# saguirregaray1/walkai-nos

Measured on AMD Instinct MI355X. Metric: aggregate GPU utilization % + schedulable pods/node, mixed fractional-GPU load, higher is better.
Workload: dtype fp32

## Files before the change

### csrc/attn_wide.hip

```cpp
#include <hip/hip_runtime.h>

#include "pin.h"
#include "x3_common.h"

#include <utility>

namespace {

template <class F, int... Q>
__device__ __forceinline__ void x3w_slots(F& f, std::integer_sequence<int, Q...>) {
  (f(std::integral_constant<int, Q>{}), ...);
}

#ifndef NOS_X3W_FENCE
#define NOS_X3W_FENCE 1
#endif
__device__ __forceinline__ f32x16 x3_step(int k, const bf16x8& a0, const bf16x8& a1, const bf16x8& a2,
                                          const bf16x8& b0, const bf16x8& b1, const bf16x8& b2, const f32x16& d) {
  switch (k) {
    case 0: return __builtin_amdgcn_mfma_f32_32x32x16_bf16(a2, b0, d, 0, 0, 0);
    case 1: return __builtin_amdgcn_mfma_f32_32x32x16_bf16(a1, b1, d, 0, 0, 0);
    case 2: return __builtin_amdgcn_mfma_f32_32x32x16_bf16(a0, b2, d, 0, 0, 0);
    case 3: return __builtin_amdgcn_mfma_f32_32x32x16_bf16(a1, b0, d, 0, 0, 0);
    case 4: return __builtin_amdgcn_mfma_f32_32x32x16_bf16(a0, b1, d, 0, 0, 0);
    default: return __builtin_amdgcn_mfma_f32_32x32x16_bf16(a0, b0, d, 0, 0, 0);
  }
}

template <bool FDIV = false>
__global__ __launch_bounds__(256, 1) void attn_fwd_x3w(const float* __restrict__ qkv, float* __restrict__ out,
                                                       __bf16* __restrict__ outp, float* __restrict__ part_o,
                                                       float* __restrict__ part_ml, int B, int T, int H, int h0,
                                                       int Ht, float scale_log2e, int Pk, int* __restrict__ cnt,
                                                       int q0, int Tq) {
  constexpr int G = 8;
  __shared__ __attribute__((aligned(16))) __bf16 lds_k[2 * 3 * XK_PLANE];
  __shared__ __attribute__((aligned(16))) __bf16 lds_v[2 * 3 * XV_PLANE];
  __shared__ int s_last;
  const int P = Pk & 0x3fffff;
  const PinnedBlock pb = pinned_block(unsigned(Pk >> 22) & 0xffu);
  if (pb.id < 0 || pb.id >= P) return;
  const int w = (Pk >> 30) ? pb.id : xcd_major_n(pb.id, P, pb.nx);
  const int NK = (T + 31) / 32, QT = (Tq + 31) / 32, QG = (QT + G - 1) / G;
  const long long U = (long long)B * H * QG * NK;
  const float rP = FDIV ? 1.f / float(P) : 0.f, rNK = FDIV ? 1.f / float(NK) : 0.f;
  const float rQG = FDIV ? 1.f / float(QG) : 0.f, rH = FDIV ? 1.f / float(H) : 0.f;
  long long u = FDIV ? udiv23(w * U, P, rP) : sk_begin(w, U, P);
  const long long u1 = FDIV ? udiv23((w + 1) * U, P, rP) : sk_begin(w + 1, U, P);
  const int D = Ht * HD, ld = 3 * D;
  const int tid = threadIdx.x, lane = tid & 63;
  const int wv = __builtin_amdgcn_readfirstlane(tid >> 6);
  const int j = lane & 31, hf = lane >> 5;
  const int lrow = tid >> 3, lch = tid & 7;
  const int gi = lane & 15, gg = lane >> 4;
  const int vtr = (4 * hf + (gi >> 2)) * XV_STR + 16 * (gg & 1) + 4 * (gi & 3);
  bool first = true;
  while (u < u1) {
    const long long grp = FDIV ? udiv23(u, NK, rNK) : u / NK;
    const int kb0 = int(u - grp * NK);
    const int kb1 = int(min<long long>(NK, kb0 + (u1 - u)));
    const int nb = kb1 - kb0;
    const long long gq = FDIV ? udiv23(grp, QG, rQG) : grp / QG;
    const int qg = int(grp - gq * QG);
    const long long bq = FDIV ? udiv23(gq, H, rH) : gq / H;
    const int head = h0 + int(gq - bq * H);
    const int b = int(bq);
    const float* basef = qkv + size_t(b) * T * ld;
    const int qtA = qg * G + 2 * wv, qtB = qtA + 1;
    const bool activeA = qtA < QT, activeB = qtB < QT;

    bf16x8 qa[3][4], qb[3][4];
    {
      const float* qpa = basef + size_t(q0 + min(qtA * 32 + j, Tq - 1)) * ld + head * HD + 8 * hf;
      const float* qpb = basef + size_t(q0 + min(qtB * 32 + j, Tq - 1)) * ld + head * HD + 8 * hf;
#pragma unroll
      for (int s = 0; s < 4; ++s) {
        const f32x4 alo = *reinterpret_cast<const f32x4*>(qpa + 16 * s);
        const f32x4 ahi = *reinterpret_cast<const f32x4*>(qpa + 16 * s + 4);
        const f32x4 blo = *reinterpret_cast<const f32x4*>(qpb + 16 * s);
        const f32x4 bhi = *reinterpret_cast<const f32x4*>(qpb + 16 * s + 4);
        split3(f32x8{alo[0], alo[1], alo[2], alo[3], ahi[0], ahi[1], ahi[2], ahi[3]}, qa[0][s], qa[1][s], qa[2][s]);
        split3(f32x8{blo[0], blo[1], blo[2], blo[3], bhi[0], bhi[1], bhi[2], bhi[3]}, qb[0][s], qb[1][s], qb[2][s]);
      }
#pragma unroll
      for (int p = 0; p < 3; ++p)
#pragma unroll
        for (int s = 0; s < 4; ++s) asm volatile("" : "+a"(qa[p][s]), "+a"(qb[p][s]));
    }
    const float* kgf = basef + D + head * HD + 8 * lch;
    const float* vgf = basef + 2 * D + head * HD + 8 * lch;
    f32x4 fk0, fk1, fv0, fv1;
    auto fetch_k = [&](int blk) {
      const size_t r = size_t(min(blk * 32 + lrow, T - 1)) * ld;
      fk0 = *reinterpret_cast<const f32x4*>(kgf + r);
      fk1 = *reinterpret_cast<const f32x4*>(kgf + r + 4);
    };
    auto fetch_v = [&](int blk) {
      const size_t r = size_t(min(blk * 32 + lrow, T - 1)) * ld;
      fv0 = *reinterpret_cast<const f32x4*>(vgf + r);
      fv1 = *reinterpret_cast<const f32x4*>(vgf + r + 4);
    };
    auto stash = [](const f32x4& lo, const f32x4& hi, __bf16* d, int pstride) {
      bf16x8 a0, a1, a2;
      split3(f32x8{lo[0], lo[1], lo[2], lo[3], hi[0], hi[1], hi[2], hi[3]}, a0, a1, a2);
      *reinterpret_cast<bf16x8*>(d) = a0;
      *reinterpret_cast<bf16x8*>(d + pstride) = a1;
      *reinterpret_cast<bf16x8*>(d + 2 * pstride) = a2;
    };
    auto stash_k = [&](int buf) { stash(fk0, fk1, &lds_k[buf * 3 * XK_PLANE + lrow * XK_STR + 8 * lch], XK_PLANE); };
    auto stash_v = [&](int buf) { stash(fv0, fv1, &lds_v[buf * 3 * XV_PLANE + lrow * XV_STR + 8 * lch], XV_PLANE); };
    auto qk_all = [&](f32x16& SA, f32x16& SB, int buf) {
      const __bf16* ks_ = &lds_k[buf * 3 * XK_PLANE + j * XK_STR + 8 * hf];
      SA = f32x16{0};
      SB = f32x16{0};
#pragma unroll
      for (int s = 0; s < 4; ++s) {
        const bf16x8 k0 = *reinterpret_cast<const bf16x8*>(ks_ + 16 * s);
        const bf16x8 k1 = *reinterpret_cast<const bf16x8*>(ks_ + XK_PLANE + 16 * s);
        const bf16x8 k2 = *reinterpret_cast<const bf16x8*>(ks_ + 2 * XK_PLANE + 16 * s);
        SA = mfma_x3(k0, k1, k2, qa[0][s], qa[1][s], qa[2][s], SA);
        SB = mfma_x3(k0, k1, k2, qb[0][s], qb[1][s], qb[2][s], SB);
      }
    };
    auto rowmax = [&](const f32x16& S) {
      float mx = fmaxf(S[0], S[1]);
#pragma unroll
      for (int r = 2; r < 16; ++r) mx = fmaxf(mx, S[r]);
      return half_max(mx);
    };
    __syncthreads();
    fetch_k(kb0);
    fetch_v(kb0);
    stash_k(0);
    stash_v(0);
    fetch_k(kb0 + 1);
    stash_k(1);
    __syncthreads();
    f32x16 oa0 = {0}, oa1 = {0}, ob0 = {0}, ob1 = {0}, sca, scb, sna, snb;
    float ma = -INFINITY, la = 0.f, mb = -INFINITY, lb = 0.f;
    qk_all(sca, scb, 0);
    float mxa = rowmax(sca), mxb = rowmax(scb);
    __syncthreads();
    auto rescale = [&](float mx, float& m, float& l, f32x16& o0, f32x16& o1) {
      if (__builtin_amdgcn_ballot_w64((mx - m) * scale_log2e > 8.f)) {
        const float m_new = fmaxf(m, mx);
        const float alpha = __builtin_amdgcn_exp2f((m - m_new) * scale_log2e);
        l *= alpha;
        o0 *= alpha;
        o1 *= alpha;
        m = m_new;
      }
    };
    auto iter = [&](f32x16& SA, f32x16& SB, f32x16& NA, f32x16& NB, float& mxA, float& mxB, int i) {
      const int blk = kb0 + i;
      if (blk * 32 + 32 > T) {
        asm volatile("; tail block: mask keys >= T" ::: "memory");
#pragma unroll
        for (int r = 0; r < 16; ++r)
          if (blk * 32 + key_of(r, hf) >= T) SA[r] = SB[r] = -INFINITY;
        mxA = rowmax(SA);
        mxB = rowmax(SB);
      }
      rescale(mxA, ma, la, oa0, oa1);
      rescale(mxB, mb, lb, ob0, ob1);
      fetch_k(blk + 2);
      fetch_v(blk + 1);
      const float mcA = ma * scale_log2e, mcB = mb * scale_log2e;
      float psA = 0.f, psB = 0.f;
      const __bf16* ks_ = &lds_k[((i + 1) & 1) * 3 * XK_PLANE + j * XK_STR + 8 * hf];
      const __bf16* vs_ = &lds_v[(i & 1) * 3 * XV_PLANE + vtr];
      bf16x8 kf[2][3], vf[2][2][3];
      uint32_t pw[2][2][3][4];
      float ra[2], rb[2];
      typedef float f32x2v __attribute__((ext_vector_type(2)));
      typedef __bf16 bf16x2v __attribute__((ext_vector_type(2)));
      bf16x2v kh[3][4], vh[3][4];
      f32x2v kr[4], vr[4];
      float mxn = 0.f;
      auto read_k = [&](int s, int slot) {
#pragma unroll
        for (int p = 0; p < 3; ++p) kf[slot][p] = *reinterpret_cast<const bf16x8*>(ks_ + p * XK_PLANE + 16 * s);
      };
      auto read_v = [&](int s2, int dh, int p) {
        const __bf16* a = vs_ + p * XV_PLANE + 16 * s2 * XV_STR + 32 * dh;
        const bf16x4 lo = __builtin_amdgcn_ds_read_tr16_b64_v4bf16((lds_bf16x4*)(a));
        const bf16x4 hi = __builtin_amdgcn_ds_read_tr16_b64_v4bf16((lds_bf16x4*)(a + 8 * XV_STR));
        vf[s2][dh][p] = bf16x8{lo[0], lo[1], lo[2], lo[3], hi[0], hi[1], hi[2], hi[3]};
      };
      auto expo = [&](int t, int r) {
        if (t)
          SB[r] = __builtin_amdgcn_exp2f(fmaf(SB[r], scale_log2e, -mcB));
        else
          SA[r] = __builtin_amdgcn_exp2f(fmaf(SA[r], scale_log2e, -mcA));
      };
      auto addp = [&](int t, int r) {
        if (t)
          psB += SB[r];
        else
          psA += SA[r];
      };
      auto split_a = [&](int t, int s2, int q) {
        const float a = t ? SB[8 * s2 + 2 * q] : SA[8 * s2 + 2 * q];
        const float b = t ? SB[8 * s2 + 2 * q + 1] : SA[8 * s2 + 2 * q + 1];
        const uint32_t ua = __float_as_uint(a), ub = __float_as_uint(b);
        pw[t][s2][0][q] = __builtin_amdgcn_perm(ub, ua, 0x07060302u);
        ra[t] = a - __uint_as_float(ua & 0xffff0000u);
        rb[t] = b - __uint_as_float(ub & 0xffff0000u);
      };
      auto split_b = [&](int t, int s2, int q) {
        const uint32_t ura = __float_as_uint(ra[t]), urb = __float_as_uint(rb[t]);
        pw[t][s2][1][q] = __builtin_amdgcn_perm(urb, ura, 0x07060302u);
        const float sa = ra[t] - __uint_as_float(ura & 0xffff0000u), sb = rb[t] - __uint_as_float(urb & 0xffff0000u);
        pw[t][s2][2][q] = __builtin_amdgcn_perm(__float_as_uint(sb), __float_as_uint(sa), 0x07060302u);
      };
      auto pplane = [&](int t, int s2, int p) {
        return __builtin_bit_cast(bf16x8, (uint4){pw[t][s2][p][0], pw[t][s2][p][1], pw[t][s2][p][2], pw[t][s2][p][3]});
      };
      auto stash_a = [&](bool isv, int q) {
        const f32x4 lo = isv ? fv0 : fk0, hi = isv ? fv1 : fk1;
        const f32x2v x = q < 2 ? f32x2v{lo[2 * q], lo[2 * q + 1]} : f32x2v{hi[2 * q - 4], hi[2 * q - 3]};
        const bf16x2v h0 = __builtin_convertvector(x, bf16x2v);
        const f32x2v r = x - __builtin_convertvector(h0, f32x2v);
        if (isv) vh[0][q] = h0, vr[q] = r;
        else kh[0][q] = h0, kr[q] = r;
      };
      auto stash_b = [&](bool isv, int q) {
        const f32x2v r = isv ? vr[q] : kr[q];
        const bf16x2v h1 = __builtin_convertvector(r, bf16x2v);
        const bf16x2v h2 = __builtin_convertvector(r - __builtin_convertvector(h1, f32x2v), bf16x2v);
        if (isv) vh[1][q] = h1, vh[2][q] = h2;
        else kh[1][q] = h1, kh[2][q] = h2;
      };
      auto stash_w = [&](bool isv) {
        if (isv) {
          __bf16* d = &lds_v[((i + 1) & 1) * 3 * XV_PLANE + lrow * XV_STR + 8 * lch];
#pragma unroll
          for (int p = 0; p < 3; ++p)
            *reinterpret_cast<bf16x8*>(d + p * XV_PLANE) = bf16x8{vh[p][0][0], vh[p][0][1], vh[p][1][0], vh[p][1][1],
                                                                  vh[p][2][0], vh[p][2][1], vh[p][3][0], vh[p][3][1]};
        } else {
          __bf16* d = &lds_k[(i & 1) * 3 * XK_PLANE + lrow * XK_STR + 8 * lch];
#pragma unroll
          for (int p = 0; p < 3; ++p)
            *reinterpret_cast<bf16x8*>(d + p * XK_PLANE) = bf16x8{kh[p][0][0], kh[p][0][1], kh[p][1][0], kh[p][1][1],
                                                                  kh[p][2][0], kh[p][2][1], kh[p][3][0], kh[p][3][1]};
        }
      };
      read_k(0, 0);
      __builtin_amdgcn_sched_barrier(0);
      auto slot = [&](auto qc) {
        constexpr int q = decltype(qc)::value;
        if constexpr (q < 48) {
          constexpr int s = q / 12, t = (q / 6) & 1, k = q % 6;
          const bf16x8* kk = kf[s & 1];
          const bool init = s == 0 && k == 0;
          if (t == 0)
            NA = x3_step(k, kk[0], kk[1], kk[2], qa[0][s], qa[1][s], qa[2][s], init ? f32x16{0} : NA);
          else
            NB = x3_step(k, kk[0], kk[1], kk[2], qb[0][s], qb[1][s], qb[2][s], init ? f32x16{0} : NB);
        } else {
          const int v = q - 48, s2 = v / 24, dh = (v / 12) & 1, t = (v / 6) & 1, k = v % 6;
          const bf16x8* vv = vf[s2][dh];
          const bf16x8 p0 = pplane(t, s2, 0), p1 = pplane(t, s2, 1), p2 = pplane(t, s2, 2);
          if (dh == 0 && t == 0) oa0 = x3_step(k, vv[0], vv[1], vv[2], p0, p1, p2, oa0);
          else if (dh == 0) ob0 = x3_step(k, vv[0], vv[1], vv[2], p0, p1, p2, ob0);
          else if (t == 0) oa1 = x3_step(k, vv[0], vv[1], vv[2], p0, p1, p2, oa1);
          else ob1 = x3_step(k, vv[0], vv[1], vv[2], p0, p1, p2, ob1);
        }
        if constexpr ((q >= 1 && q <= 16) || (q >= 33 && q <= 48)) {
          constexpr int e = q <= 16 ? q - 1 : q - 33;
          addp(e / 8, (q <= 16 ? 0 : 8) + e % 8);
        }
        if (q < 8) expo(0, q);
        else if (q < 16) expo(1, q - 8);
        else if (q < 32) {
          const int t = (q - 16) / 8, pq = ((q - 16) % 8) / 2;
          if (q % 2 == 0) split_a(t, 0, pq); else split_b(t, 0, pq);
        } else if (q < 40) expo(0, q - 32 + 8);
        else if (q < 48) expo(1, q - 40 + 8);
        else if (q < 64) {
          const int t = (q - 48) / 8, pq = ((q - 48) % 8) / 2;
          if (q % 2 == 0) split_a(t, 1, pq); else split_b(t, 1, pq);
        } else if (q == 64) la += half_sum(psA);
        else if (q == 65) lb += half_sum(psB);
        else if (q >= 66 && q < 70) {
          const int c = q - 66;
          float m4 = fmaxf(NA[4 * c], NA[4 * c + 1]);
          m4 = fmaxf(m4, NA[4 * c + 2]);
          m4 = fmaxf(m4, NA[4 * c + 3]);
          mxn = c ? fmaxf(mxn, m4) : m4;
        } else if (q == 70) mxA = half_max(mxn);
        else if (q >= 72 && q < 76) {
          const int c = q - 72;
          float m4 = fmaxf(NB[4 * c], NB[4 * c + 1]);
          m4 = fmaxf(m4, NB[4 * c + 2]);
          m4 = fmaxf(m4, NB[4 * c + 3]);
          mxn = c ? fmaxf(mxn, m4) : m4;
        } else if (q == 76) mxB = half_max(mxn);
        else if (q >= 77 && q < 85) {
          if ((q - 77) % 2 == 0) stash_a(false, (q - 77) / 2); else stash_b(false, (q - 77) / 2);
        } else if (q >= 86 && q < 94) {
          if ((q - 86) % 2 == 0) stash_a(true, (q - 86) / 2); else stash_b(true, (q - 86) / 2);
        }
        if (q == 2 || q == 14 || q == 26) read_k(q / 12 + 1, (q / 12 + 1) & 1);
        if (q >= 29 && q < 41 && (q - 29) % 2 == 0) read_v(0, (q - 29) / 6, (q - 29) / 2 % 3);
        if (q >= 50 && q < 62 && (q - 50) % 2 == 0) read_v(1, (q - 50) / 6, (q - 50) / 2 % 3);
        if (q == 85) stash_w(false);
        if (q == 94) stash_w(true);
        if (NOS_X3W_FENCE) __builtin_amdgcn_sched_barrier(0);
      };
      x3w_slots(slot, std::make_integer_sequence<int, 96>{});
    };
    int i = 0;
    for (; i + 1 < nb; i += 2) {
      iter(sca, scb, sna, snb, mxa, mxb, i);
      __syncthreads();
      iter(sna, snb, sca, scb, mxa, mxb, i + 1);
      __syncthreads();
    }
    if (i < nb) {
      iter(sca, scb, sna, snb, mxa, mxb, i);
      __syncthreads();
    }

    const bool whole = kb0 == 0 && kb1 == NK;
    auto store_tile = [&](int t, const f32x16& o0, const f32x16& o1, float l) {
      const int q = (qg * G + 2 * wv + t) * 32 + j;
      if (q >= Tq) return;
      const float inv = 1.f / l;
      const size_t orow = (size_t(b) * Tq + q) * D + head * HD;
      if (outp) {
        const size_t op = size_t(B) * Tq * D;
#pragma unroll
        for (int r = 0; r < 16; ++r) {
          const int d = key_of(r, hf);
          store_x3(outp, op, orow + d, o0[r] * inv);
          store_x3(outp, op, orow + 32 + d, o1[r] * inv);
        }
      } else {
#pragma unroll
        for (int r = 0; r < 16; ++r) {
          const int d = key_of(r, hf);
          out[orow + d] = o0[r] * inv;
          out[orow + 32 + d] = o1[r] * inv;
        }
      }
    };
    auto finish = [&](bool active, int t, const f32x16& o0, const f32x16& o1, float m, float l) {
      if (!active) return;
      if (whole) {
        store_tile(t, o0, o1, l);
      } else {
        const size_t slot = (size_t(w) * 2 + (first ? 0 : 1)) * G + 2 * wv + t;
        float* po = part_o + slot * (HD * 32);
#pragma unroll
        for (int r = 0; r < 16; ++r) {
          const int d = key_of(r, hf);
          po[d * 32 + j] = o0[r];
          po[(32 + d) * 32 + j] = o1[r];
        }
        if (hf == 0) {
          part_ml[slot * 64 + j] = m * scale_log2e;
          part_ml[slot * 64 + 32 + j] = l;
        }
      }
    };
    finish(activeA, 0, oa0, oa1, ma, la);
    finish(activeB, 1, ob0, ob1, mb, lb);
    if (!whole && cnt) {
      const long long t0 = grp * NK, t1 = t0 + NK;
      const long long wlo = ((t0 + 1) * P + U - 1) / U - 1, whi = (t1 * P + U - 1) / U - 1;
      __threadfence();
      __syncthreads();
      if (tid == 0) {
        int n = 0;
        for (long long x = wlo; x <= whi; ++x) n += (x * U / P != (x + 1) * U / P) ? 1 : 0;
        const int last = atomicAdd(&cnt[grp], 1) == n - 1;
        if (last) atomicExch(&cnt[grp], 0);
        s_last = last;
      }
      __syncthreads();
      if (s_last) {
        __threadfence();
        auto merge = [&](int t) {
          float M = -INFINITY, L = 0.f;
          f32x16 a0 = {0}, a1 = {0};
          for (long long x = wlo; x <= whi; ++x) {
            const long long s0 = x * U / P;
            if (s0 == (x + 1) * U / P) continue;
            const size_t slot = (size_t(x) * 2 + (s0 >= t0 ? 0 : 1)) * G + 2 * wv + t;
            const float mw = part_ml[slot * 64 + j];
            if (mw == -INFINITY) continue;
            const float lw = part_ml[slot * 64 + 32 + j];
            const float* po = part_o + slot * (HD * 32);
            const float Mn = fmaxf(M, mw);
            const float so = __builtin_amdgcn_exp2f(M - Mn), sn = __builtin_amdgcn_exp2f(mw - Mn);
            L = fmaf(lw, sn, L * so);
#pragma unroll
            for (int r = 0; r < 16; ++r) {
              const int d = key_of(r, hf);
              a0[r] = fmaf(po[d * 32 + j], sn, a0[r] * so);
              a1[r] = fmaf(po[(32 + d) * 32 + j], sn, a1[r] * so);
            }
            M = Mn;
          }
          store_tile(t, a0, a1, L);
        };
        if (activeA) merge(0);
        if (activeB) merge(1);
      }
    }
    u += kb1 - kb0;
    first = false;
  }
}

}

int nos_attn_x3w_launch(bool fdiv, dim3 grid, hipStream_t s, const float* qkv, float* out, __bf16* outp,
                        float* part_o, float* part_ml, int B, int T, int H, int h0, int Ht, float scale_log2e,
                        int Pk, int* cnt, int q0, int Tq) {
  if (fdiv)
    hipLaunchKernelGGL(attn_fwd_x3w<true>, grid, dim3(256), 0, s, qkv, out, outp, part_o, part_ml, B, T, H, h0, Ht,
                       scale_log2e, Pk, cnt, q0, Tq);
  else
    hipLaunchKernelGGL(attn_fwd_x3w<false>, grid, dim3(256), 0, s, qkv, out, outp, part_o, part_ml, B, T, H, h0, Ht,
                       scale_log2e, Pk, cnt, q0, Tq);
  return int(hipPeekAtLastError());
}

int nos_attn_x3w_occupancy() {
  int n = 0;
  if (hipOccupancyMaxActiveBlocksPerMultiprocessor(&n, attn_fwd_x3w<true>, 256, 0) != hipSuccess || n <= 0) n = 1;
  return n;
}
```

### csrc/attn_x3.hip

```cpp
#include <hip/hip_runtime.h>

#include "attn_x3.h"
#include "err.h"
#include "pin.h"
#include "x3_common.h"

#include <cmath>
#include <cstdint>
#include <cstdlib>
#include <string>

namespace {


__device__ __forceinline__ void split3_trunc8(const f32x16& acc, int e0, bf16x8& p0, bf16x8& p1, bf16x8& p2) {
  uint32_t w0[4], w1[4], w2[4];
#pragma unroll
  for (int i = 0; i < 4; ++i) {
    const float a = acc[e0 + 2 * i], b = acc[e0 + 2 * i + 1];
    const uint32_t ua = __float_as_uint(a), ub = __float_as_uint(b);
    w0[i] = __builtin_amdgcn_perm(ub, ua, 0x07060302u);
    const float ra = a - __uint_as_float(ua & 0xffff0000u), rb = b - __uint_as_float(ub & 0xffff0000u);
    const uint32_t ura = __float_as_uint(ra), urb = __float_as_uint(rb);
    w1[i] = __builtin_amdgcn_perm(urb, ura, 0x07060302u);
// ... 51 lines not shown
    uint4 pk0, pk1, pk2, pv0, pv1, pv2;
    auto fetch = [&](int blk) {
      const size_t r = size_t(min(blk * 32 + lrow, T - 1)) * ld;
      pk0 = *reinterpret_cast<const uint4*>(kg + r);
      pk1 = *reinterpret_cast<const uint4*>(kg + plane + r);
      pk2 = *reinterpret_cast<const uint4*>(kg + 2 * plane + r);
      pv0 = *reinterpret_cast<const uint4*>(vg + r);
      pv1 = *reinterpret_cast<const uint4*>(vg + plane + r);
      pv2 = *reinterpret_cast<const uint4*>(vg + 2 * plane + r);
    };
    auto stash = [&](int buf) {
      __bf16* kd = &lds_k[buf * 3 * XK_PLANE + lrow * XK_STR + 8 * lch];
      __bf16* vd = &lds_v[buf * 3 * XV_PLANE + lrow * XV_STR + 8 * lch];
      *reinterpret_cast<uint4*>(kd) = pk0;
      *reinterpret_cast<uint4*>(kd + XK_PLANE) = pk1;
      *reinterpret_cast<uint4*>(kd + 2 * XK_PLANE) = pk2;
      *reinterpret_cast<uint4*>(vd) = pv0;
      *reinterpret_cast<uint4*>(vd + XV_PLANE) = pv1;
      *reinterpret_cast<uint4*>(vd + 2 * XV_PLANE) = pv2;
    };
    __syncthreads();
    fetch(kb0);
    stash(0);
    __syncthreads();

    f32x16 o0 = {0}, o1 = {0};
    float m = -INFINITY, l = 0.f;
    for (int blk = kb0; blk < kb1; ++blk) {
      const int buf = (blk - kb0) & 1;
      const bool more = blk + 1 < kb1;
      if (more) fetch(blk + 1);
#define X3_ATTN_BLOCK(MASKED)                                                                        \
  {                                                                                                  \
    const __bf16* ks = &lds_k[buf * 3 * XK_PLANE + j * XK_STR + 8 * hf];                             \
    f32x16 sacc = {0};                                                                               \
    _Pragma("unroll") for (int s = 0; s < 4; ++s) {                                                  \
      const bf16x8 k0 = *reinterpret_cast<const bf16x8*>(ks + 16 * s);                               \
      const bf16x8 k1 = *reinterpret_cast<const bf16x8*>(ks + XK_PLANE + 16 * s);                     \
      const bf16x8 k2 = *reinterpret_cast<const bf16x8*>(ks + 2 * XK_PLANE + 16 * s);                 \
      sacc = mfma_x3(k0, k1, k2, qf[0][s], qf[1][s], qf[2][s], sacc);                                \
    }                                                                                                \
    if (MASKED) {                                                                                    \
      asm volatile("; tail block: mask keys >= T" ::: "memory");           \
      _Pragma("unroll") for (int r = 0; r < 16; ++r) if (blk * 32 + key_of(r, hf) >= T) sacc[r] = -INFINITY; \
    }                                                                                                \
    float mx = fmaxf(sacc[0], sacc[1]);                                                              \
    _Pragma("unroll") for (int r = 2; r < 16; ++r) mx = fmaxf(mx, sacc[r]);                          \
    mx = half_max(mx);                                                          \
    if (__builtin_amdgcn_ballot_w64((mx - m) * scale_log2e > 8.f)) {                                 \
      const float m_new = fmaxf(m, mx);                                                              \
      const float alpha = __builtin_amdgcn_exp2f((m - m_new) * scale_log2e);                         \
      l *= alpha;                                                                                    \
      o0 *= alpha;                                                                                   \
      o1 *= alpha;                                                                                   \
      m = m_new;                                                                                     \
    }                                                                                                \
    const float mc = m * scale_log2e;                                                                \
    float psum = 0.f;                                                                                \
    _Pragma("unroll") for (int r = 0; r < 16; ++r) {                                                 \
      sacc[r] = __builtin_amdgcn_exp2f(fmaf(sacc[r], scale_log2e, -mc));                             \
      psum += sacc[r];                                                                               \
    }                                                                                                \
    psum = half_sum(psum);                                                                \
    l += psum;                                                                                       \
    const __bf16* vs = &lds_v[buf * 3 * XV_PLANE + vtr];                                             \
    _Pragma("unroll") for (int s2 = 0; s2 < 2; ++s2) {                                               \
      bf16x8 p0, p1, p2;                                                                             \
      split3_trunc8(sacc, 8 * s2, p0, p1, p2);                                                       \
      _Pragma("unroll") for (int dh = 0; dh < 2; ++dh) {                                             \
        bf16x8 vf[3];                                                                                \
        _Pragma("unroll") for (int p = 0; p < 3; ++p) {                                              \
          const __bf16* a = vs + p * XV_PLANE + 16 * s2 * XV_STR + 32 * dh;                          \
          const bf16x4 lo = __builtin_amdgcn_ds_read_tr16_b64_v4bf16((lds_bf16x4*)(a));              \
          const bf16x4 hi = __builtin_amdgcn_ds_read_tr16_b64_v4bf16((lds_bf16x4*)(a + 8 * XV_STR)); \
          vf[p] = bf16x8{lo[0], lo[1], lo[2], lo[3], hi[0], hi[1], hi[2], hi[3]};                    \
        }                                                                                            \
        if (dh == 0)                                                                                 \
          o0 = mfma_x3(vf[0], vf[1], vf[2], p0, p1, p2, o0);                                         \
        else                                                                                         \
          o1 = mfma_x3(vf[0], vf[1], vf[2], p0, p1, p2, o1);                                         \
      }                                                                                              \
    }                                                                                                \
  }
      if (active) X3_ATTN_BLOCK(blk * 32 + 32 > T)
#undef X3_ATTN_BLOCK
      if (more) stash(buf ^ 1);
      __syncthreads();
    }

    if (active) {
      if (kb0 == 0 && kb1 == NK) {
        const int q = q0 + j;
        if (q < T) {
          const float inv = 1.f / l;
          const size_t orow = (size_t(b) * T + q) * D + head * HD;
          if (outp) {
            const size_t op = size_t(B) * T * D;
#pragma unroll
            for (int r = 0; r < 16; ++r) {
              const int d = key_of(r, hf);
              store_x3(outp, op, orow + d, o0[r] * inv);
              store_x3(outp, op, orow + 32 + d, o1[r] * inv);
            }
          } else {
#pragma unroll
            for (int r = 0; r < 16; ++r) {
              const int d = key_of(r, hf);
              out[orow + d] = o0[r] * inv;
              out[orow + 32 + d] = o1[r] * inv;
            }
          }
        }
      } else {
        const size_t slot = (size_t(w) * 2 + (first ? 0 : 1)) * 4 + wv;
        float* po = part_o + slot * (HD * 32);
#pragma unroll
        for (int r = 0; r < 16; ++r) {
          const int d = key_of(r, hf);
          po[d * 32 + j] = o0[r];
          po[(32 + d) * 32 + j] = o1[r];
        }
        if (hf == 0) {
          part_ml[slot * 64 + j] = m * scale_log2e;
          part_ml[slot * 64 + 32 + j] = l;
        }
      }
    }
    u += kb1 - kb0;
    first = false;
  }
}

template <int G, bool QW = false, bool F32IN = false, bool PRIO = false, bool FDIV = false>
__global__ __launch_bounds__(64 * G, 8 / G) void attn_fwd_x3p(const __bf16* __restrict__ qkv3, size_t plane,
                                                             float* __restrict__ out, __bf16* __restrict__ outp,
                                                             float* __restrict__ part_o, float* __restrict__ part_ml,
                                                             int B, int T, int H, int h0, int Ht, float scale_log2e,
                                                             int Pk, int qw0, int Tq) {
  static_assert(G == 4 || G == 8, "4 or 8 query tiles per workgroup");
  __shared__ __attribute__((aligned(16))) __bf16 lds_k[2 * 3 * XK_PLANE];
  __shared__ __attribute__((aligned(16))) __bf16 lds_v[2 * 3 * XV_PLANE];
  const int P = Pk & 0x3fffff;
  const PinnedBlock pb = pinned_block(unsigned(Pk >> 22) & 0xffu);
  if (pb.id < 0 || pb.id >= P) return;
  const int w = (Pk >> 30) ? pb.id : xcd_major_n(pb.id, P, pb.nx);
  const int NK = (T + 31) / 32, QT = (Tq + 31) / 32, QG = (QT + G - 1) / G;
  const long long U = (long long)B * H * QG * NK;
  const float rP = FDIV ? 1.f / float(P) : 0.f, rNK = FDIV ? 1.f / float(NK) : 0.f;
  const float rQG = FDIV ? 1.f / float(QG) : 0.f, rH = FDIV ? 1.f / float(H) : 0.f;
  long long u = FDIV ? udiv23(w * U, P, rP) : sk_begin(w, U, P);
  const long long u1 = FDIV ? udiv23((w + 1) * U, P, rP) : sk_begin(w + 1, U, P);
  const int D = Ht * HD, ld = 3 * D;
  const int tid = threadIdx.x, wv = tid >> 6, lane = tid & 63;
  const int j = lane & 31, hf = lane >> 5;
  const int lrow = (tid & 255) >> 3, lch = tid & 7;
  const bool kload = G == 4 || tid < 256;
  const bool vload = G == 4 || tid >= 256;
  const int gi = lane & 15, gg = lane >> 4;
  const int vtr = (4 * hf + (gi >> 2)) * XV_STR + 16 * (gg & 1) + 4 * (gi & 3);
  bool first = true;
  while (u < u1) {
    const long long grp = FDIV ? udiv23(u, NK, rNK) : u / NK;
    const int kb0 = int(u - grp * NK);
    const int kb1 = int(min<long long>(NK, kb0 + (u1 - u)));
    const int nb = kb1 - kb0;
    const long long gq = FDIV ? udiv23(grp, QG, rQG) : grp / QG;
    const int qg = int(grp - gq * QG);
    const long long bq = FDIV ? udiv23(gq, H, rH) : gq / H;
    const int head = h0 + int(gq - bq * H);
    const int b = int(bq);
    const __bf16* base = qkv3 + size_t(b) * T * ld;
    const float* basef = reinterpret_cast<const float*>(qkv3) + size_t(b) * T * ld;
    const int qt = qg * G + wv;
    const bool active = qt < QT;
    const int q0 = qt * 32;

    bf16x8 qf[3][4];
    {
      const int qrow = qw0 + min(q0 + j, Tq - 1);
      if constexpr (F32IN) {
        const float* qp = basef + size_t(qrow) * ld + head * HD + 8 * hf;
#pragma unroll
        for (int s = 0; s < 4; ++s) {
          const f32x4 lo = *reinterpret_cast<const f32x4*>(qp + 16 * s);
          const f32x4 hi = *reinterpret_cast<const f32x4*>(qp + 16 * s + 4);
          const f32x8 x = {lo[0], lo[1], lo[2], lo[3], hi[0], hi[1], hi[2], hi[3]};
          split3(x, qf[0][s], qf[1][s], qf[2][s]);
        }
      } else {
        const __bf16* qp = base + size_t(qrow) * ld + head * HD + 8 * hf;
#pragma unroll
        for (int p = 0; p < 3; ++p)
#pragma unroll
          for (int s = 0; s < 4; ++s) qf[p][s] = *reinterpret_cast<const bf16x8*>(qp + p * plane + 16 * s);
      }
    }
    const __bf16* kg = base + D + head * HD + 8 * lch;
    const __bf16* vg = base + 2 * D + head * HD + 8 * lch;
    const float* kgf = basef + D + head * HD + 8 * lch;
    const float* vgf = basef + 2 * D + head * HD + 8 * lch;
    uint4 pk0, pk1, pk2, pv0, pv1, pv2;
    f32x4 fk0, fk1, fv0, fv1;
    auto fetch_k = [&](int blk) {
      const size_t r = size_t(min(blk * 32 + lrow, T - 1)) * ld;
      if constexpr (F32IN) {
        fk0 = *reinterpret_cast<const f32x4*>(kgf + r);
        fk1 = *reinterpret_cast<const f32x4*>(kgf + r + 4);
      } else {
        pk0 = *reinterpret_cast<const uint4*>(kg + r);
        pk1 = *reinterpret_cast<const uint4*>(kg + plane + r);
        pk2 = *reinterpret_cast<const uint4*>(kg + 2 * plane + r);
      }
    };
    auto fetch_v = [&](int blk) {
      const size_t r = size_t(min(blk * 32 + lrow, T - 1)) * ld;
      if constexpr (F32IN) {
        fv0 = *reinterpret_cast<const f32x4*>(vgf + r);
        fv1 = *reinterpret_cast<const f32x4*>(vgf + r + 4);
      } else {
        pv0 = *reinterpret_cast<const uint4*>(vg + r);
        pv1 = *reinterpret_cast<const uint4*>(vg + plane + r);
        pv2 = *reinterpret_cast<const uint4*>(vg + 2 * plane + r);
      }
    };
    auto split_chunk = [](const f32x4& lo, const f32x4& hi, uint4& c0, uint4& c1, uint4& c2) {
      const f32x8 x = {lo[0], lo[1], lo[2], lo[3], hi[0], hi[1], hi[2], hi[3]};
      bf16x8 a0, a1, a2;
      split3(x, a0, a1, a2);
      c0 = __builtin_bit_cast(uint4, a0), c1 = __builtin_bit_cast(uint4, a1), c2 = __builtin_bit_cast(uint4, a2);
    };
    auto stash_k = [&](int buf) {
      if constexpr (F32IN) split_chunk(fk0, fk1, pk0, pk1, pk2);
      __bf16* kd = &lds_k[buf * 3 * XK_PLANE + lrow * XK_STR + 8 * lch];
      *reinterpret_cast<uint4*>(kd) = pk0;
      *reinterpret_cast<uint4*>(kd + XK_PLANE) = pk1;
      *reinterpret_cast<uint4*>(kd + 2 * XK_PLANE) = pk2;
    };
    auto stash_v = [&](int buf) {
      if constexpr (F32IN) split_chunk(fv0, fv1, pv0, pv1, pv2);
      __bf16* vd = &lds_v[buf * 3 * XV_PLANE + lrow * XV_STR + 8 * lch];
      *reinterpret_cast<uint4*>(vd) = pv0;
      *reinterpret_cast<uint4*>(vd + XV_PLANE) = pv1;
      *reinterpret_cast<uint4*>(vd + 2 * XV_PLANE) = pv2;
    };
#define X3P_QK(SACC, BUF)                                                                        \
  {                                                                                              \
    const __bf16* ks_ = &lds_k[(BUF) * 3 * XK_PLANE + j * XK_STR + 8 * hf];                      \
    SACC = f32x16{0};                                                                            \
    _Pragma("unroll") for (int s = 0; s < 4; ++s) {                                              \
      const bf16x8 k0 = *reinterpret_cast<const bf16x8*>(ks_ + 16 * s);                           \
      const bf16x8 k1 = *reinterpret_cast<const bf16x8*>(ks_ + XK_PLANE + 16 * s);                 \
      const bf16x8 k2 = *reinterpret_cast<const bf16x8*>(ks_ + 2 * XK_PLANE + 16 * s);             \
      SACC = mfma_x3(k0, k1, k2, qf[0][s], qf[1][s], qf[2][s], SACC);                            \
    }                                                                                            \
  }
    __syncthreads();
    if (kload) {
      fetch_k(kb0);
      stash_k(0);
      if (nb > 1) {
        fetch_k(kb0 + 1);
        stash_k(1);
      }
    }
    if (vload) {
      fetch_v(kb0);
      stash_v(0);
    }
    __syncthreads();

    if constexpr (QW) __builtin_amdgcn_s_waitcnt(0xF70);
    f32x16 o0 = {0}, o1 = {0}, scur = {0};
    float m = -INFINITY, l = 0.f;
    if (active) X3P_QK(scur, 0)
    __syncthreads();
#define X3P_PV(VB)                                                                                        \
  {                                                                                                       \
    const __bf16* vs_ = &lds_v[(VB) * 3 * XV_PLANE + vtr];                                                \
    _Pragma("unroll") for (int s2 = 0; s2 < 2; ++s2) {                                                    \
      _Pragma("unroll") for (int dh = 0; dh < 2; ++dh) {                                                  \
        bf16x8 vf[3];                                                                                     \
        _Pragma("unroll") for (int p = 0; p < 3; ++p) {                                                   \
          const __bf16* a = vs_ + p * XV_PLANE + 16 * s2 * XV_STR + 32 * dh;                              \
          const bf16x4 lo = __builtin_amdgcn_ds_read_tr16_b64_v4bf16((lds_bf16x4*)(a));                   \
          const bf16x4 hi = __builtin_amdgcn_ds_read_tr16_b64_v4bf16((lds_bf16x4*)(a + 8 * XV_STR));      \
          vf[p] = bf16x8{lo[0], lo[1], lo[2], lo[3], hi[0], hi[1], hi[2], hi[3]};                         \
        }                                                                                                 \
        const bf16x8 q0_ = s2 ? pb0 : pa0;                                                                \
        const bf16x8 q1_ = s2 ? pb1 : pa1;                                                                \
        const bf16x8 q2_ = s2 ? pb2 : pa2;                                                                \
        if (dh == 0)                                                                                      \
          o0 = mfma_x3(vf[0], vf[1], vf[2], q0_, q1_, q2_, o0);                                           \
        else                                                                                              \
          o1 = mfma_x3(vf[0], vf[1], vf[2], q0_, q1_, q2_, o1);                                           \
      }                                                                                                   \
    }                                                                                                     \
  }
#define X3P_ITER(SC, SN)                                                                                  \
  {                                                                                                       \
      const int blk = kb0 + i;                                                                            \
      const bool more_k = i + 2 < nb, more_v = i + 1 < nb;                                                \
      if (kload && more_k) fetch_k(blk + 2);                                                                      \
      if (vload && more_v) fetch_v(blk + 1);                                                                      \
      if (active) {                                                                                       \
        if (blk * 32 + 32 > T) {                                                                          \
          asm volatile("; tail block: mask keys >= T" ::: "memory");                                      \
          _Pragma("unroll") for (int r = 0; r < 16; ++r)                                                  \
            if (blk * 32 + key_of(r, hf) >= T) SC[r] = -INFINITY;                                         \
        }                                                                                                 \
        float mx = fmaxf(SC[0], SC[1]);                                                                   \
        _Pragma("unroll") for (int r = 2; r < 16; ++r) mx = fmaxf(mx, SC[r]);                             \
        mx = half_max(mx);                                                                                \
        if (__builtin_amdgcn_ballot_w64((mx - m) * scale_log2e > 8.f)) {                                  \
          const float m_new = fmaxf(m, mx);                                                               \
          const float alpha = __builtin_amdgcn_exp2f((m - m_new) * scale_log2e);                          \
          l *= alpha;                                                                                     \
          o0 *= alpha;                                                                                    \
          o1 *= alpha;                                                                                    \
          m = m_new;                                                                                      \
        }                                                                                                 \
                 X3P_QK(SN, (i + 1) & 1)                                                                   \
        const float mc = m * scale_log2e;                                                                 \
        float psum = 0.f;                                                                                 \
        _Pragma("unroll") for (int r = 0; r < 16; ++r) {                                                  \
          SC[r] = __builtin_amdgcn_exp2f(fmaf(SC[r], scale_log2e, -mc));                                  \
          psum += SC[r];                                                                                  \
        }                                                                                                 \
        psum = half_sum(psum);                                                                            \
        l += psum;                                                                                        \
        const __bf16* vs = &lds_v[(i & 1) * 3 * XV_PLANE + vtr];                                          \
        _Pragma("unroll") for (int s2 = 0; s2 < 2; ++s2) {                                                \
          bf16x8 p0, p1, p2;                                                                              \
          split3_trunc8(SC, 8 * s2, p0, p1, p2);                                                          \
          _Pragma("unroll") for (int dh = 0; dh < 2; ++dh) {                                              \
            bf16x8 vf[3];                                                                                 \
            _Pragma("unroll") for (int p = 0; p < 3; ++p) {                                               \
              const __bf16* a = vs + p * XV_PLANE + 16 * s2 * XV_STR + 32 * dh;                           \
              const bf16x4 lo = __builtin_amdgcn_ds_read_tr16_b64_v4bf16((lds_bf16x4*)(a));               \
              const bf16x4 hi = __builtin_amdgcn_ds_read_tr16_b64_v4bf16((lds_bf16x4*)(a + 8 * XV_STR));  \
              vf[p] = bf16x8{lo[0], lo[1], lo[2], lo[3], hi[0], hi[1], hi[2], hi[3]};                     \
            }                                                                                             \
            if (dh == 0)                                                                                  \
              o0 = mfma_x3(vf[0], vf[1], vf[2], p0, p1, p2, o0);                                          \
            else                                                                                          \
              o1 = mfma_x3(vf[0], vf[1], vf[2], p0, p1, p2, o1);                                          \
          }                                                                                               \
        }                                                                                                 \
      }                                                                                                   \
      if (kload && more_k) stash_k(i & 1);                                                                 \
      if (vload && more_v) stash_v((i + 1) & 1);                                                           \
      __syncthreads();                                                                                    \
  }
#define X3P_ITER_LATE(SC, SN)                                                                                  \
  {                                                                                                       \
      const int blk = kb0 + i;                                                                            \
      const bool more_k = i + 2 < nb, more_v = i + 1 < nb;                                                \
      if (kload && more_k) fetch_k(blk + 2);                                                                      \
      if (vload && more_v) fetch_v(blk + 1);                                                                      \
      if (active) {                                                                                       \
        if (i > 0) X3P_PV((i - 1) & 1)    \
        if (blk * 32 + 32 > T) {                                                                          \
          asm volatile("; tail block: mask keys >= T" ::: "memory");                                      \
          _Pragma("unroll") for (int r = 0; r < 16; ++r)                                                  \
            if (blk * 32 + key_of(r, hf) >= T) SC[r] = -INFINITY;                                         \
        }                                                                                                 \
        float mx = fmaxf(SC[0], SC[1]);                                                                   \
        _Pragma("unroll") for (int r = 2; r < 16; ++r) mx = fmaxf(mx, SC[r]);                             \
        mx = half_max(mx);                                                                                \
        if (__builtin_amdgcn_ballot_w64((mx - m) * scale_log2e > 8.f)) {                                  \
          const float m_new = fmaxf(m, mx);                                                               \
          const float alpha = __builtin_amdgcn_exp2f((m - m_new) * scale_log2e);                          \
          l *= alpha;                                                                                     \
          o0 *= alpha;                                                                                    \
          o1 *= alpha;                                                                                    \
          m = m_new;                                                                                      \
        }                                                                                                 \
                 X3P_QK(SN, (i + 1) & 1)                                                                   \
        const float mc = m * scale_log2e;                                                                 \
        float psum = 0.f;                                                                                 \
        _Pragma("unroll") for (int r = 0; r < 16; ++r) {                                                  \
          SC[r] = __builtin_amdgcn_exp2f(fmaf(SC[r], scale_log2e, -mc));                                  \
          psum += SC[r];                                                                                  \
        }                                                                                                 \
        psum = half_sum(psum);                                                                            \
        l += psum;                                                                                        \
        split3_trunc8(SC, 0, pa0, pa1, pa2);                                                              \
        split3_trunc8(SC, 8, pb0, pb1, pb2);                                                              \
      }                                                                                                   \
      if (kload && more_k) stash_k(i & 1);                                                                 \
      if (vload && more_v) stash_v((i + 1) & 1);                                                           \
      __syncthreads();                                                                                    \
  }
    f32x16 snext;
    bf16x8 pa0, pa1, pa2, pb0, pb1, pb2;
    if constexpr (PRIO) {
      if (G == 8 && wv >= 4) __builtin_amdgcn_s_setprio(1);
    }
    if (G == 8 && wv >= 4) {
      for (int i = 0; i < nb;) {
        X3P_ITER_LATE(scur, snext)
        if (++i >= nb) break;
        X3P_ITER_LATE(snext, scur)
        ++i;
      }
      if (active && nb > 0) X3P_PV((nb - 1) & 1)
    } else {
      for (int i = 0; i < nb;) {
        X3P_ITER(scur, snext)
        if (++i >= nb) break;
        X3P_ITER(snext, scur)
        ++i;
      }
    }
#undef X3P_ITER
#undef X3P_ITER_LATE
#undef X3P_PV
#undef X3P_QK

    if (active) {
      if (kb0 == 0 && kb1 == NK) {
        const int q = q0 + j;
        if (q < Tq) {
          const float inv = 1.f / l;
          const size_t orow = (size_t(b) * Tq + q) * D + head * HD;
          if (outp) {
            const size_t op = size_t(B) * Tq * D;
#pragma unroll
            for (int r = 0; r < 16; ++r) {
              const int d = key_of(r, hf);
              store_x3(outp, op, orow + d, o0[r] * inv);
              store_x3(outp, op, orow + 32 + d, o1[r] * inv);
            }
          } else {
#pragma unroll
            for (int r = 0; r < 16; ++r) {
              const int d = key_of(r, hf);
              out[orow + d] = o0[r] * inv;
              out[orow + 32 + d] = o1[r] * inv;
            }
          }
        }
      } else {
        const size_t slot = (size_t(w) * 2 + (first ? 0 : 1)) * G + wv;
        float* po = part_o + slot * (HD * 32);
#pragma unroll
        for (int r = 0; r < 16; ++r) {
          const int d = key_of(r, hf);
          po[d * 32 + j] = o0[r];
          po[(32 + d) * 32 + j] = o1[r];
        }
        if (hf == 0) {
          part_ml[slot * 64 + j] = m * scale_log2e;
          part_ml[slot * 64 + 32 + j] = l;
        }
      }
    }
    u += kb1 - kb0;
    first = false;
  }
}


template <int G>
__global__ __launch_bounds__(256) void attn_sk_lds_fixup(const float* __restrict__ part_o,
                                                         const float* __restrict__ part_ml, float* __restrict__ out,
                                                         int B, int T, int H, int P, __bf16* __restrict__ outp,
                                                         int h0, int Ht, unsigned pin, int Tq) {
  __shared__ float s_tile[64][33];
  const int NK = (T + 31) / 32, QT = (Tq + 31) / 32, QG = (QT + G - 1) / G;
  const long long U = (long long)B * H * QG * NK;
  const bool narrow_stores = (pin >> 8) & 1u;
  const bool xcd_local = (pin >> 9) & 1u;
  pin &= 0xffu;
  const PinnedBlock pb = pinned_block(pin);
  if (pb.id < 0) return;
  const int R = B * H * QG;
  int id0 = pb.id, idn = R * G, step = pb.n, base = 0;
  if (xcd_local && !pin) {
    const int x = int(blockIdx.x) % 8, qq = P / 8, rr = P % 8;
    auto rlo = [&](int xx) -> int {
      if (xx >= 8) return R;
      const long long ws = (long long)xx * qq + min(xx, rr);
      const long long num = ws * U + 1 - P, den = (long long)NK * P;
      const long long r0 = num <= 0 ? 0 : (num + den - 1) / den;
      return int(min<long long>(r0, R));
    };
    const int r0 = rlo(x), r1 = rlo(x + 1);
    base = r0 * G;
    idn = max(0, r1 - r0) * G;
    id0 = int(blockIdx.x) / 8;
    step = int(gridDim.x) / 8;
  }
  for (int id_ = id0; id_ < idn; id_ += step) {
  const int id = base + id_;
  const int wv = id % G;
  const long long grp = id / G;
  const int qg = int(grp % QG);
  const int qt = qg * G + wv;
  if (qt >= QT) continue;
  const long long t0 = grp * NK, t1 = t0 + NK;
  const long long w_lo = ((t0 + 1) * P + U - 1) / U - 1;
  const long long w_hi = (t1 * P + U - 1) / U - 1;
  if (w_lo == w_hi) continue;
  const int head = h0 + int((grp / QG) % H);
  const int b = int(grp / ((long long)QG * H));
  const int D = Ht * HD;
  const int tid = threadIdx.x;
  auto slot_of = [&](long long w) -> long long {
    const long long s = w * U / P;
    if (s == (w + 1) * U / P) return -1;
    return (w * 2 + (s >= t0 ? 0 : 1)) * G + wv;
  };
  const int q = tid & 31;
  float M = -INFINITY, L = 0.f;
  float acc[8];
#pragma unroll
  for (int i = 0; i < 8; ++i) acc[i] = 0.f;
  for (long long w0 = w_lo; w0 <= w_hi; w0 += 4) {
    float mw[4], lw[4], ow[4][8];
#pragma unroll
    for (int c = 0; c < 4; ++c) {
      const long long w = w0 + c;
      const long long sl = w <= w_hi ? slot_of(w) : -1;
      mw[c] = -INFINITY;
      lw[c] = 0.f;
#pragma unroll
      for (int i = 0; i < 8; ++i) ow[c][i] = 0.f;
      if (sl >= 0) {
        mw[c] = part_ml[sl * 64 + q];
        lw[c] = part_ml[sl * 64 + 32 + q];
        const float* po = part_o + sl * (HD * 32);
#pragma unroll
        for (int i = 0; i < 8; ++i) ow[c][i] = po[tid + 256 * i];
      }
    }
#pragma unroll
    for (int c = 0; c < 4; ++c) {
      if (mw[c] == -INFINITY) continue;
      const float Mn = fmaxf(M, mw[c]);
      const float so = __builtin_amdgcn_exp2f(M - Mn), sn = __builtin_amdgcn_exp2f(mw[c] - Mn);
      L = fmaf(lw[c], sn, L * so);
#pragma unroll
      for (int i = 0; i < 8; ++i) acc[i] = fmaf(ow[c][i], sn, acc[i] * so);
      M = Mn;
    }
  }
  const float inv = 1.f / L;
#pragma unroll
  for (int i = 0; i < 8; ++i) s_tile[(tid + 256 * i) >> 5][q] = acc[i] * inv;
  __syncthreads();
  const size_t plane = size_t(B) * Tq * D;
  if (!narrow_stores) {
    const int jq = tid >> 3, c8 = 8 * (tid & 7);
    const int qq = qt * 32 + jq;
    if (qq < Tq) {
      const size_t i = (size_t(b) * Tq + qq) * D + head * HD + c8;
      f32x8 v;
#pragma unroll
      for (int dd = 0; dd < 8; ++dd) v[dd] = s_tile[c8 + dd][jq];
      if (outp) {
        bf16x8 p0, p1, p2;
        split3(v, p0, p1, p2);
        *reinterpret_cast<bf16x8*>(outp + i) = p0;
        *reinterpret_cast<bf16x8*>(outp + plane + i) = p1;
        *reinterpret_cast<bf16x8*>(outp + 2 * plane + i) = p2;
      } else {
        *reinterpret_cast<f32x4*>(out + i) = f32x4{v[0], v[1], v[2], v[3]};
        *reinterpret_cast<f32x4*>(out + i + 4) = f32x4{v[4], v[5], v[6], v[7]};
      }
    }
  } else {
  const int d = tid & 63;
  for (int jq = tid >> 6; jq < 32; jq += 4) {
    const int qq = qt * 32 + jq;
    if (qq >= Tq) break;
    const size_t i = (size_t(b) * Tq + qq) * D + head * HD + d;
    if (outp)
      store_x3(outp, plane, i, s_tile[d][jq]);
    else
      out[i] = s_tile[d][jq];
  }
  }
  __syncthreads();
  }
}

}

extern "C" {

static int g_x3_pipelined = 1;
static int g_x3_flags = 0;

int nos_attention_x3_set_flags(int f) {
  g_x3_flags = f;
  return 0;
}
static int g_x3_group = 8;
static int g_x3_wide = [] {
  const char* e = std::getenv("NOS_ATTN_WIDE");
  return (e && std::string(e) == "0") ? 0 : 1;
}();

int nos_attention_x3_set_wide(int on) {
  g_x3_wide = on ? 1 : 0;
  return 0;
}

int nos_attention_x3_wide() { return g_x3_wide; }

int nos_attention_x3_pipelined() { return g_x3_pipelined; }

int nos_attention_x3_set_group(int g) {
  if (g != 4 && g != 8) {
    nos_kernels_set_error("attention x3: group must be 4 or 8");
    return -1;
  }
  g_x3_group = g;
  return 0;
}

int nos_attention_x3_group() { return g_x3_pipelined ? g_x3_group : 4; }

int nos_attention_x3_set_pipelined(int on) {
  g_x3_pipelined = on ? 1 : 0;
  return 0;
}

int nos_attention_x3_wg_per_cu() {
  if (g_x3_pipelined && g_x3_group == 8 && g_x3_wide) return nos_attn_x3w_occupancy();
  int n = 0;
  const hipError_t e =
      !g_x3_pipelined  ? hipOccupancyMaxActiveBlocksPerMultiprocessor(&n, attn_fwd_x3, 256, 0)
      : g_x3_group == 8 ? hipOccupancyMaxActiveBlocksPerMultiprocessor(&n, attn_fwd_x3p<8>, 512, 0)
                        : hipOccupancyMaxActiveBlocksPerMultiprocessor(&n, attn_fwd_x3p<4>, 256, 0);
  if (e != hipSuccess || n <= 0) n = 1;
  return n;
}

int nos_attention_x3(const NosAttnX3* a, void* stream) {
  const auto fail = [](const char* msg) {
    nos_kernels_set_error(msg);
    return -1;
  };
  if (a == nullptr || a->size != int(sizeof(NosAttnX3)))
    return fail("attention x3: launch descriptor of another size (NosAttnX3, csrc/attn_x3.h)");
  const int B = a->B, T = a->T, H = a->H, h0 = a->h0, hn = a->hn, waves = a->waves, q0 = a->q0, Tq = a->Tq;
  const bool f32in = a->f32in != 0, fixup = a->fixup != 0;
  float* const out = a->out;
  int* const cnt = a->cnt;
  if (q0 < 0 || Tq <= 0 || (long long)q0 + Tq > T)
    return fail("attention x3: query window out of range (needs q0 >= 0, Tq > 0, q0 + Tq <= T)");
  const bool windowed = q0 != 0 || Tq != T;
  if (windowed && (!g_x3_pipelined || cnt != nullptr || !fixup))
    return fail("attention x3: a query window needs the pipelined kernel and the separate fixup launch");
  if (cnt != nullptr && (long long)a->ncnt < (long long)B * hn * (((T + 31) / 32 + 7) / 8))
    return fail("attention x3 merged: needs B*hn*QG row counters");
  if ((out == nullptr) == (a->outp == nullptr)) return fail("attention x3: exactly one of out / outp");
  if (!fixup && out == nullptr) return fail("attention x3 partials: needs the fp32 direct-output buffer");
  if (a->head_dim != HD) return fail("attention x3: head_dim must be 64");
  if (a->ws == nullptr || waves <= 0) return fail("attention x3: needs waves > 0 and a workspace");
  if (!f32in && a->plane_stride % 8)
    return fail("attention x3: plane stride must be a multiple of 8 elements (16-B aligned planes)");
  if (h0 < 0 || hn <= 0 || h0 + hn > H) return fail("attention x3: head block out of range");
  if (!g_x3_pipelined && (h0 != 0 || hn != H)) return fail("attention x3: head blocks need the pipelined kernel");
  if (f32in && (!g_x3_pipelined || nos_attention_x3_group() != 8))
    return fail("attention x3: fp32 input needs the pipelined 8-tile kernel");
  hipStream_t s = reinterpret_cast<hipStream_t>(stream);
  const int G = nos_attention_x3_group();
  const int NK = (T + 31) / 32, QT = (Tq + 31) / 32, QG = (QT + G - 1) / G;
  float* part_o = a->ws;
  float* part_ml = a->ws + size_t(waves) * 2 * G * HD * 32;
  __bf16* op = reinterpret_cast<__bf16*>(a->outp);
  const float sl2 = a->scale * 1.4426950408889634f;
  const __bf16* q3 = reinterpret_cast<const __bf16*>(a->qkv);
  const size_t plane_stride = f32in ? 0 : a->plane_stride;
  if (waves >= (1 << 22)) return fail("attention x3: at most 2^22 workgroups");
  const unsigned pin = nos_pin_mask();
  if (pin && !g_x3_pipelined) return fail("attention x3: pinned launches need the pipelined kernel");
  const int pk = waves | int(pin << 22) | ((g_x3_flags & 4) ? (1 << 30) : 0);
  const long long Uk = (long long)B * hn * QG * NK;
  const bool fdiv = !(g_x3_flags & 8) && (Uk + 1) * (waves + 1) < (1ll << 23);
  const dim3 grid(pinned_grid(waves, pin));
  const auto x3p = [&](auto kernel, int block) {
    hipLaunchKernelGGL(kernel, grid, dim3(block), 0, s, q3, plane_stride, out, op, part_o, part_ml, B, T, hn, h0, H,
                       sl2, pk, q0, Tq);
  };
  if (!g_x3_pipelined)
    hipLaunchKernelGGL(attn_fwd_x3, dim3(waves), dim3(256), 0, s, q3, plane_stride, out, op, part_o, part_ml, B, T, H,
                       sl2, waves);
  else if (G == 8 && f32in && g_x3_wide)
    nos_attn_x3w_launch(fdiv, grid, s, reinterpret_cast<const float*>(a->qkv), out, op, part_o, part_ml, B, T, hn, h0,
                        H, sl2, pk, fixup ? cnt : nullptr, q0, Tq);
  else if (G == 8 && f32in && (g_x3_flags & 2))
    x3p(attn_fwd_x3p<8, false, true, true>, 512);
  else if (G == 8 && f32in && fdiv)
    x3p(attn_fwd_x3p<8, false, true, false, true>, 512);
// ... 29 lines not shown
```

Measured before the change: 335.2.

## Triple-buffer K in LDS and prefetch next K fragment across iterations

The wide attention kernel moves from double to triple buffering of the split-bf16 K tiles in LDS, with rotating read/write/next offsets. The first K fragment of the next block is read from LDS in the middle of the current iteration, and the global fetches of V and K are pushed later in the slot schedule. The rescale-needed ballot is computed ahead of time, and the mxB and stash slots are shifted earlier. In the x3 kernel, the PV step moves ahead of the active branch, and extra syncthreads are added for partially idle late waves. The aim is to hide LDS and global load latency behind the MFMA work, at the cost of more LDS use and register pressure.

```diff
diff --git a/csrc/attn_wide.hip b/csrc/attn_wide.hip
--- a/csrc/attn_wide.hip
+++ b/csrc/attn_wide.hip
@@ -15,6 +15,7 @@
 #ifndef NOS_X3W_FENCE
 #define NOS_X3W_FENCE 1
 #endif
+constexpr int X3W_KBUFS = 3;
 __device__ __forceinline__ f32x16 x3_step(int k, const bf16x8& a0, const bf16x8& a1, const bf16x8& a2,
                                           const bf16x8& b0, const bf16x8& b1, const bf16x8& b2, const f32x16& d) {
   switch (k) {
@@ -34,7 +35,7 @@
                                                        int Ht, float scale_log2e, int Pk, int* __restrict__ cnt,
                                                        int q0, int Tq) {
   constexpr int G = 8;
-  __shared__ __attribute__((aligned(16))) __bf16 lds_k[2 * 3 * XK_PLANE];
+  __shared__ __attribute__((aligned(16))) __bf16 lds_k[X3W_KBUFS * 3 * XK_PLANE];
   __shared__ __attribute__((aligned(16))) __bf16 lds_v[2 * 3 * XV_PLANE];
   __shared__ int s_last;
   const int P = Pk & 0x3fffff;
@@ -135,14 +136,25 @@
     stash_v(0);
     fetch_k(kb0 + 1);
     stash_k(1);
+    fetch_k(kb0 + 2);
+    stash_k(2);
     __syncthreads();
     f32x16 oa0 = {0}, oa1 = {0}, ob0 = {0}, ob1 = {0}, sca, scb, sna, snb;
     float ma = -INFINITY, la = 0.f, mb = -INFINITY, lb = 0.f;
     qk_all(sca, scb, 0);
     float mxa = rowmax(sca), mxb = rowmax(scb);
+    int k_wr = 0, k_rd = 3 * XK_PLANE, k_nx = 6 * XK_PLANE;
+    bf16x8 kpre[3];
+#pragma unroll
+    for (int p = 0; p < 3; ++p)
+      kpre[p] = *reinterpret_cast<const bf16x8*>(&lds_k[k_rd + p * XK_PLANE + j * XK_STR + 8 * hf]);
+    auto need = [&](float mx, float m) { return __builtin_amdgcn_ballot_w64((mx - m) * scale_log2e > 8.f) != 0; };
+    bool needA = need(mxa, ma), needB = need(mxb, mb);
+    fetch_k(kb0 + 3);
+    fetch_v(kb0 + 1);
     __syncthreads();
-    auto rescale = [&](float mx, float& m, float& l, f32x16& o0, f32x16& o1) {
-      if (__builtin_amdgcn_ballot_w64((mx - m) * scale_log2e > 8.f)) {
+    auto rescale = [&](bool nd, float mx, float& m, float& l, f32x16& o0, f32x16& o1) {
+      if (nd) {
         const float m_new = fmaxf(m, mx);
         const float alpha = __builtin_amdgcn_exp2f((m - m_new) * scale_log2e);
         l *= alpha;
@@ -160,14 +172,14 @@
           if (blk * 32 + key_of(r, hf) >= T) SA[r] = SB[r] = -INFINITY;
         mxA = rowmax(SA);
         mxB = rowmax(SB);
-      }
-      rescale(mxA, ma, la, oa0, oa1);
-      rescale(mxB, mb, lb, ob0, ob1);
-      fetch_k(blk + 2);
-      fetch_v(blk + 1);
+        needA = need(mxA, ma);
+        needB = need(mxB, mb);
+      }
+      rescale(needA, mxA, ma, la, oa0, oa1);
+      rescale(needB, mxB, mb, lb, ob0, ob1);
       const float mcA = ma * scale_log2e, mcB = mb * scale_log2e;
       float psA = 0.f, psB = 0.f;
-      const __bf16* ks_ = &lds_k[((i + 1) & 1) * 3 * XK_PLANE + j * XK_STR + 8 * hf];
+      const __bf16* ks_ = &lds_k[k_rd + j * XK_STR + 8 * hf];
       const __bf16* vs_ = &lds_v[(i & 1) * 3 * XV_PLANE + vtr];
       bf16x8 kf[2][3], vf[2][2][3];
       uint32_t pw[2][2][3][4];
@@ -239,14 +251,15 @@
             *reinterpret_cast<bf16x8*>(d + p * XV_PLANE) = bf16x8{vh[p][0][0], vh[p][0][1], vh[p][1][0], vh[p][1][1],
                                                                   vh[p][2][0], vh[p][2][1], vh[p][3][0], vh[p][3][1]};
         } else {
-          __bf16* d = &lds_k[(i & 1) * 3 * XK_PLANE + lrow * XK_STR + 8 * lch];
+          __bf16* d = &lds_k[k_wr + lrow * XK_STR + 8 * lch];
 #pragma unroll
           for (int p = 0; p < 3; ++p)
             *reinterpret_cast<bf16x8*>(d + p * XK_PLANE) = bf16x8{kh[p][0][0], kh[p][0][1], kh[p][1][0], kh[p][1][1],
                                                                   kh[p][2][0], kh[p][2][1], kh[p][3][0], kh[p][3][1]};
         }
       };
-      read_k(0, 0);
+#pragma unroll
+      for (int p = 0; p < 3; ++p) kf[0][p] = kpre[p];
       __builtin_amdgcn_sched_barrier(0);
       auto slot = [&](auto qc) {
         constexpr int q = decltype(qc)::value;
@@ -290,26 +303,38 @@
           m4 = fmaxf(m4, NA[4 * c + 3]);
           mxn = c ? fmaxf(mxn, m4) : m4;
         } else if (q == 70) mxA = half_max(mxn);
-        else if (q >= 72 && q < 76) {
-          const int c = q - 72;
+        else if (q >= 71 && q < 75) {
+          const int c = q - 71;
           float m4 = fmaxf(NB[4 * c], NB[4 * c + 1]);
           m4 = fmaxf(m4, NB[4 * c + 2]);
           m4 = fmaxf(m4, NB[4 * c + 3]);
           mxn = c ? fmaxf(mxn, m4) : m4;
-        } else if (q == 76) mxB = half_max(mxn);
-        else if (q >= 77 && q < 85) {
-          if ((q - 77) % 2 == 0) stash_a(false, (q - 77) / 2); else stash_b(false, (q - 77) / 2);
-        } else if (q >= 86 && q < 94) {
-          if ((q - 86) % 2 == 0) stash_a(true, (q - 86) / 2); else stash_b(true, (q - 86) / 2);
+        } else if (q == 75) mxB = half_max(mxn);
+        else if (q >= 76 && q < 84) {
+          if ((q - 76) % 2 == 0) stash_a(false, (q - 76) / 2); else stash_b(false, (q - 76) / 2);
+        } else if (q >= 84 && q < 92) {
+          if ((q - 84) % 2 == 0) stash_a(true, (q - 84) / 2); else stash_b(true, (q - 84) / 2);
+        } else if (q == 93) fetch_v(blk + 2);
+        else if (q == 94) fetch_k(blk + 4);
+        else if (q == 95) {
+          needA = need(mxA, ma);
+          needB = need(mxB, mb);
         }
         if (q == 2 || q == 14 || q == 26) read_k(q / 12 + 1, (q / 12 + 1) & 1);
         if (q >= 29 && q < 41 && (q - 29) % 2 == 0) read_v(0, (q - 29) / 6, (q - 29) / 2 % 3);
         if (q >= 50 && q < 62 && (q - 50) % 2 == 0) read_v(1, (q - 50) / 6, (q - 50) / 2 % 3);
-        if (q == 85) stash_w(false);
-        if (q == 94) stash_w(true);
+        if (q == 62) {
+#pragma unroll
+          for (int p = 0; p < 3; ++p)
+            kpre[p] = *reinterpret_cast<const bf16x8*>(&lds_k[k_nx + p * XK_PLANE + j * XK_STR + 8 * hf]);
+        }
+        if (q == 84) stash_w(false);
+        if (q == 92) stash_w(true);
         if (NOS_X3W_FENCE) __builtin_amdgcn_sched_barrier(0);
       };
       x3w_slots(slot, std::make_integer_sequence<int, 96>{});
+      const int t = k_wr;
+      k_wr = k_rd, k_rd = k_nx, k_nx = t;
     };
     int i = 0;
     for (; i + 1 < nb; i += 2) {
diff --git a/csrc/attn_x3.hip b/csrc/attn_x3.hip
--- a/csrc/attn_x3.hip
+++ b/csrc/attn_x3.hip
@@ -377,6 +377,7 @@
       const bool more_k = i + 2 < nb, more_v = i + 1 < nb;                                                \
       if (kload && more_k) fetch_k(blk + 2);                                                                      \
       if (vload && more_v) fetch_v(blk + 1);                                                                      \
+      if (late_idle && i > 0) __syncthreads();                                                           \
       if (active) {                                                                                       \
         if (blk * 32 + 32 > T) {                                                                          \
           asm volatile("; tail block: mask keys >= T" ::: "memory");                                      \
@@ -432,8 +433,9 @@
       const bool more_k = i + 2 < nb, more_v = i + 1 < nb;                                                \
       if (kload && more_k) fetch_k(blk + 2);                                                                      \
       if (vload && more_v) fetch_v(blk + 1);                                                                      \
+      if (active && i > 0) X3P_PV((i - 1) & 1)  \
+      if (late_idle && i > 0) __syncthreads();                                                           \
       if (active) {                                                                                       \
-        if (i > 0) X3P_PV((i - 1) & 1)    \
         if (blk * 32 + 32 > T) {                                                                          \
           asm volatile("; tail block: mask keys >= T" ::: "memory");                                      \
           _Pragma("unroll") for (int r = 0; r < 16; ++r)                                                  \
@@ -468,6 +470,7 @@
   }
     f32x16 snext;
     bf16x8 pa0, pa1, pa2, pb0, pb1, pb2;
+    const bool late_idle = G == 8 && QT - qg * G > 4 && QT - qg * G < 8;
     if constexpr (PRIO) {
       if (G == 8 && wv >= 4) __builtin_amdgcn_s_setprio(1);
     }
```

After: 325.1. -3.0%, worse.
